# flanggut/smvs

Hardware: NVIDIA H100
Metric: Gauss-Newton Mpix-iters/sec (higher is better)
Workload: dtype f64

## Files before the change

### smvs_b200/csrc/api.cu

```cuda
#include <algorithm>
#include <atomic>
#include <cmath>
#include <cstring>
#include <dlfcn.h>

#include "common.cuh"

namespace smvsb {
std::atomic<uint64_t> g_launches(0);
std::atomic<uint64_t> g_device_launches[SMVSB_MAX_DEVICES];
}

namespace {

thread_local std::string g_last_error = "";

void
quiesce (smvsb_ctx* ctx)
{
    if (ctx == nullptr)
        return;
    if (ctx->copy_stream) cudaStreamSynchronize(ctx->copy_stream);
    if (ctx->stream) cudaStreamSynchronize(ctx->stream);
}
// ... 184 lines not shown
        c->have_color = false;
    }
    for (int k = 0; c->have_color && k < n_sub; ++k)
        if (c->subs[k].w != sub_w[k] || c->subs[k].h != sub_h[k])
            c->have_color = false;
}

void
set_neighbour_tables (smvsb_ctx* c, int n_sub, int const* sub_w,
    int const* sub_h, double const* Mi, double const* ti)
{
    c->n_sub = n_sub;
    std::vector<float const*> ptrs(std::max(n_sub, 1), nullptr);
    std::vector<int> dims(std::max(2 * n_sub, 2), 0);
    std::vector<double> mt(std::max(12 * n_sub, 12), 0.0);
    for (int k = 0; k < n_sub; ++k)
    {
        smvsb::SubViewDev& sv = c->subs[k];
        sv.w = sub_w[k]; sv.h = sub_h[k];
        sv.texels.reserve(static_cast<size_t>(sv.w) * sv.h * SMVSB_NB_STRIDE);
        ptrs[k] = sv.texels.p;
        dims[2 * k] = sv.w; dims[2 * k + 1] = sv.h;
        std::copy(Mi + 9 * k, Mi + 9 * k + 9, mt.begin() + 12 * k);
        std::copy(ti + 3 * k, ti + 3 * k + 3, mt.begin() + 12 * k + 9);
    }
    upload(c, c->sub_ptrs, ptrs.data(), ptrs.size());
    upload(c, c->sub_dims, dims.data(), dims.size());
    upload(c, c->Mt, mt.data(), mt.size());
}

void
upload_color_images (smvsb_ctx* c, float const* main_rgb,
    float const* const* sub_rgb)
{
    upload(c, c->color_main, main_rgb, static_cast<size_t>(c->w) * c->h * 3);
    std::vector<float const*> ptrs(c->n_sub);
    for (int k = 0; k < c->n_sub; ++k)
    {
        upload(c, c->color_subs[k], sub_rgb[k],
            static_cast<size_t>(c->subs[k].w) * c->subs[k].h * 3);
        ptrs[k] = c->color_subs[k].p;
    }
    upload(c, c->color_ptrs, ptrs.data(), ptrs.size());
}

void
ensure_system_buffers (smvsb_ctx* c)
{
    size_t const np = c->n_patches, nn = c->n_nodes;
    c->patch_H.reserve(np * 256);
    c->patch_g.reserve(np * 16);
    c->patch_proc.reserve(np);
    c->H.reserve(nn * 144);
    c->P.reserve(nn * 16);
    c->g.reserve(nn * 4);
    c->x.reserve(nn * 4);
    c->light.reserve(16);
}

void
set_active (smvsb_ctx* c, uint8_t const* active_nodes)
{
    if (active_nodes != nullptr)
        upload(c, c->active, active_nodes, c->n_nodes);
    else
    {
        c->active.reserve(c->n_nodes);
        CUDA_CHECK(cudaMemcpyAsync(c->active.p, c->node_valid.p, c->n_nodes,
            cudaMemcpyDeviceToDevice, c->stream));
    }
}

void
construct (smvsb_ctx* c, double const* light16, double reg, double light_reg)
{
    require(c->have_views && c->have_surface, SMVSB_ERR_STATE,
        "smvsb_set_views and smvsb_set_surface must precede construct");
    if (light16 != nullptr)
    {
        require(c->have_shading, SMVSB_ERR_STATE,
            "lighting given but the main view has no shading image");
        upload(c, c->light, light16, 16);
    }
    ensure_system_buffers(c);
    smvsb::launch_construct(c, light16 != nullptr, reg, light_reg);
    c->have_system = true;
}

void
require_surface_scale (int scale)
{
    require(scale >= 0 && scale <= SMVSB_MAX_SCALE, SMVSB_ERR_INVALID,
        "surface scale out of range (0..8)");
}

void
configure_grid (smvsb_ctx* c, int scale, int npx, int npy, int start_x,
    int start_y)
{
    require_surface_scale(scale);
    require(npx > 0 && npy > 0, SMVSB_ERR_INVALID, "empty patch grid");
    int const ps = 1 << scale;
    int const sampling = sampling_for_scale(scale);
    require(ps % sampling == 0, SMVSB_ERR_INVALID,
        "patch size below sampling");
    int const npos = ps / sampling;
    require(npos == 1 || npos == 2 || npos == 4 || npos == 8
// ... 1203 lines not shown
        {
            require(off.back() <= vis_capacity, SMVSB_ERR_INVALID,
                "vis_ids capacity too small");
            if (off.back() > 0)
                download(c, vis_ids, c->vis_ids.p, off.back());
        }
    });
}

int
smvsb_get_depth (smvsb_ctx* ctx, float* depth_wh)
{
    if (ctx == nullptr) return SMVSB_ERR_INVALID;
    return guarded(ctx, [&]() {
        require(ctx->have_surface && depth_wh, SMVSB_ERR_STATE,
            "no surface set");
        size_t const n = static_cast<size_t>(ctx->w) * ctx->h;
        ctx->image_out.reserve(n * 3);
        smvsb::launch_render_depth(ctx, ctx->image_out.p);
        download(ctx, depth_wh, ctx->image_out.p, n);
    });
}

int
smvsb_get_normals (smvsb_ctx* ctx, float* normals_wh3)
{
    if (ctx == nullptr) return SMVSB_ERR_INVALID;
    return guarded(ctx, [&]() {
        require(ctx->have_surface && normals_wh3, SMVSB_ERR_STATE,
            "no surface set");
        size_t const n = static_cast<size_t>(ctx->w) * ctx->h * 3;
        ctx->image_out.reserve(n);
        smvsb::launch_render_normals(ctx, ctx->image_out.p);
        download(ctx, normals_wh3, ctx->image_out.p, n);
    });
}

int
smvsb_debug_get_system (smvsb_ctx* ctx, double* g, double* Hvals,
    uint64_t* Houter, uint64_t* Hinner, uint64_t* nnzb_h, double* Pvals,
    uint64_t* Pouter, uint64_t* Pinner, uint64_t* nnzb_p)
{
    if (ctx == nullptr) return SMVSB_ERR_INVALID;
    return guarded(ctx, [&]() {
        smvsb_ctx* c = ctx;
        require(c->have_system, SMVSB_ERR_STATE, "no system constructed");
        int const nn = c->n_nodes, ns = c->npx + 1;
        std::vector<uint8_t> active(nn), proc(c->n_patches);
        download(c, active.data(), c->active.p, nn);
        download(c, proc.data(), c->patch_proc.p, c->n_patches);
        if (g)
            download(c, g, c->g.p, static_cast<size_t>(nn) * 4);
        std::vector<double> H, P;
        if (Hvals)
        {
            H.resize(static_cast<size_t>(nn) * 144);
            download(c, H.data(), c->H.p, H.size());
        }
        if (Pvals)
        {
            P.resize(static_cast<size_t>(nn) * 16);
            download(c, P.data(), c->P.p, P.size());
        }
        uint64_t nh = 0, np = 0;
        for (int j = 0; j < nn; ++j)
        {
            if (Houter) Houter[j] = nh;
            if (Pouter) Pouter[j] = np;
            int const jx = j % ns, jy = j / ns;
            if (!c->h_node_valid[j] || !active[j])
                continue;
            for (int dy = -1; dy <= 1; ++dy)
                for (int dx = -1; dx <= 1; ++dx)
                {
                    int const ix = jx + dx, iy = jy + dy;
                    if (ix < 0 || ix > c->npx || iy < 0 || iy > c->npy)
                        continue;
                    int const i = iy * ns + ix;
                    if (!c->h_node_valid[i] || !active[i])
                        continue;
                    bool shared = false;
                    for (int pb = 0; pb < 2 && !shared; ++pb)
                        for (int pa = 0; pa < 2 && !shared; ++pa)
                        {
                            int const px = jx - 1 + pa, py = jy - 1 + pb;
                            if (px < 0 || px >= c->npx || py < 0
                                || py >= c->npy)
                                continue;
                            if (!proc[py * c->npx + px])
                                continue;
                            if (ix >= px && ix <= px + 1 && iy >= py
                                && iy <= py + 1)
                                shared = true;
                        }
                    if (!shared)
                        continue;
                    if (Hvals)
                    {
                        int const k = (-dy + 1) * 3 + (-dx + 1);
                        std::copy(H.begin() + (static_cast<size_t>(i) * 9 + k)
                            * 16, H.begin() + (static_cast<size_t>(i) * 9 + k)
                            * 16 + 16, Hvals + nh * 16);
                    }
                    if (Hinner) Hinner[nh] = static_cast<uint64_t>(i) * 4;
                    nh += 1;
                    if (i == j)
                    {
                        if (Pvals)
                            std::copy(P.begin() + static_cast<size_t>(i) * 16,
                                P.begin() + static_cast<size_t>(i) * 16 + 16,
                                Pvals + np * 16);
                        if (Pinner) Pinner[np] = static_cast<uint64_t>(i) * 4;
                        np += 1;
                    }
                }
// ... 138 lines not shown
```

### smvs_b200/csrc/cg.cu

```cuda
#include <algorithm>

#include "common.cuh"

namespace smvsb {

namespace {

constexpr int CG_THREADS = 256;
constexpr int CG_WARPS = CG_THREADS / 32;
constexpr int CG_QUADS = CG_THREADS / 4;
constexpr int CG_MAX_BLOCKS = 1024;
constexpr int CG_UF = 4;
constexpr int CG_SLOTS = 10;
constexpr int CG_ROW_CACHE = 16;

struct CgView
{
    int n_nodes, npx;
    int grid;
    int pad;
    double err_tol;
    double const* H;
    double const* P;
    double const* g;
    uint16_t const* rowmask;
    uint32_t const* rows;
    unsigned long long const* counts;
    double* x;
    double* r;
    double* d;
    double* d2;
    double* Ad;
    double* z;
    double* partials;
    double* result;
};

struct CgArgs
{
    int n_views;
    int max_iter;
    double q_tol;
    unsigned int* sync;
    CgView v[SMVSB_MAX_BATCH];
};

struct CgState
{
    double r_dot_r, Q0, beta, alpha, tol;
    double* partials;
    int n_rows, passes, done, iters, info;
    int grid;
};

__device__ __forceinline__ void
grid_barrier (unsigned int* counter, unsigned int& epoch)
{
    __syncthreads();
    if (threadIdx.x == 0)
    {
        epoch += 1;
        unsigned int const target = epoch * gridDim.x;
        asm volatile("red.release.gpu.global.add.u32 [%0], 1;"
            :: "l"(counter) : "memory");
        unsigned int v;
        do {
            asm volatile("ld.relaxed.gpu.global.u32 %0, [%1];"
                : "=r"(v) : "l"(counter) : "memory");
        } while (v < target);
        asm volatile("ld.acquire.gpu.global.u32 %0, [%1];"
            : "=r"(v) : "l"(counter) : "memory");
    }
    __syncthreads();
}

__device__ __forceinline__ unsigned long long
policy_evict_first (void)
{
    unsigned long long pol;
    asm("createpolicy.fractional.L2::evict_first.b64 %0, 1.0;" : "=l"(pol));
    return pol;
}

__device__ __forceinline__ void
ld_stream (double const* p, double2& h01, double2& h23)
{
    unsigned long long const pol = policy_evict_first();
    asm volatile("ld.global.L1::no_allocate.L2::cache_hint.v2.f64 "
        "{%0, %1}, [%2], %3;"
        : "=d"(h01.x), "=d"(h01.y) : "l"(p), "l"(pol));
    asm volatile("ld.global.L1::no_allocate.L2::cache_hint.v2.f64 "
        "{%0, %1}, [%2], %3;"
        : "=d"(h23.x), "=d"(h23.y) : "l"(p + 2), "l"(pol));
}

__device__ __forceinline__ double2
ld_vec (double const* p)
{
    return *reinterpret_cast<double2 const*>(p);
}

__device__ __forceinline__ double2
ld_hint (double const* p, unsigned long long policy)
{
    double2 v;
    asm volatile("ld.global.L2::cache_hint.v2.f64 {%0, %1}, [%2], %3;"
        : "=d"(v.x), "=d"(v.y) : "l"(p), "l"(policy));
    return v;
}

__device__ __forceinline__ unsigned long long
policy_evict_last (void)
{
    unsigned long long pol;
    asm volatile("createpolicy.fractional.L2::evict_last.b64 %0, 1.0;"
        : "=l"(pol));
    return pol;
}

template <int NV>
__device__ __forceinline__ void
warp_flush (double (&v)[NV], double* s_red, int view)
{
#pragma unroll
    for (int j = 0; j < NV; ++j)
        for (int off = 16; off > 0; off >>= 1)
            v[j] += __shfl_down_sync(0xffffffffu, v[j], off);
    if ((threadIdx.x & 31) == 0)
    {
#pragma unroll
        for (int j = 0; j < NV; ++j)
            s_red[(view * 3 + j) * CG_WARPS + (threadIdx.x >> 5)] = v[j];
    }
}

template <int NV>
__device__ __forceinline__ void
publish (CgArgs const& a, CgState const* s_state, double const* s_red,
    int first_slot, bool init)
{
    __syncthreads();
    int const t = threadIdx.x;
    if (t < a.n_views * NV)
    {
        int const view = t / NV, j = t % NV;
        CgState const& S = s_state[view];
        if (static_cast<int>(blockIdx.x) < S.grid && (init || !S.done))
        {
            double total = 0.0;
            if (S.passes > 0)
                for (int i = 0; i < CG_WARPS; ++i)
                    total += s_red[(view * 3 + j) * CG_WARPS + i];
            S.partials[(first_slot + j) * CG_MAX_BLOCKS + blockIdx.x] = total;
        }
    }
}

template <int NV>
__device__ __forceinline__ void
all_sums (CgArgs const& a, CgState const* s_state, int first_slot,
    double* s_bcast, bool init)
{
    int const warp = threadIdx.x >> 5, lane = threadIdx.x & 31;
    for (int pair = warp; pair < a.n_views * NV; pair += CG_WARPS)
    {
        int const view = pair / NV, j = pair % NV;
        if (!init && s_state[view].done)
            continue;
        double const* p = s_state[view].partials
            + (first_slot + j) * CG_MAX_BLOCKS;
        int const nb = s_state[view].grid;
        double v = 0.0;
        for (int base = lane; base < nb; base += 32 * 12)
        {
            double t[12];
#pragma unroll
            for (int u = 0; u < 12; ++u)
                t[u] = (base + 32 * u < nb) ? __ldcg(p + base + 32 * u) : 0.0;
#pragma unroll
            for (int u = 0; u < 12; ++u)
                if (base + 32 * u < nb)
                    v += t[u];
        }
        for (int off = 16; off > 0; off >>= 1)
            v += __shfl_down_sync(0xffffffffu, v, off);
        if (lane == 0)
            s_bcast[view * 3 + j] = v;
    }
    __syncthreads();
}

struct PlainVec
{
    double const* v;
    __device__ __forceinline__ void load (int node, double* out) const
    {
        double2 const a = *reinterpret_cast<double2 const*>(
            v + static_cast<size_t>(node) * 4);
        double2 const b = *reinterpret_cast<double2 const*>(
            v + static_cast<size_t>(node) * 4 + 2);
        out[0] = a.x; out[1] = a.y; out[2] = b.x; out[3] = b.y;
    }
};

struct DirVec
{
    double const* z;
    double const* d_old;
    double beta;
    __device__ __forceinline__ void load (int node, double* out) const
    {
        double2 const z0 = ld_vec(z + static_cast<size_t>(node) * 4);
        double2 const z1 = ld_vec(z + static_cast<size_t>(node) * 4 + 2);
        double2 const d0 = ld_vec(d_old + static_cast<size_t>(node) * 4);
        double2 const d1 = ld_vec(d_old + static_cast<size_t>(node) * 4 + 2);
        out[0] = z0.x + d0.x * beta; out[1] = z0.y + d0.y * beta;
        out[2] = z1.x + d1.x * beta; out[3] = z1.y + d1.y * beta;
    }
};

struct StreamRows
{
    double const* H;
    __device__ __forceinline__ double const* row (int node, int rp) const
    {
        return H + static_cast<size_t>(node) * 144 + rp * 4;
    }
    __device__ __forceinline__ void load (double const* p, double2& h01,
        double2& h23) const
    {
        ld_stream(p, h01, h23);
    }
};

constexpr int CG_PIN_STRIDE = 146;
constexpr size_t CG_PIN_BYTES = sizeof(double) * CG_PIN_STRIDE * CG_QUADS;

struct PinnedRows
{
    double const* s;
    __device__ __forceinline__ double const* row (int, int rp) const
    {
        return s + (threadIdx.x >> 2) * CG_PIN_STRIDE + rp * 4;
    }
    __device__ __forceinline__ void load (double const* p, double2& h01,
        double2& h23) const
    {
        h01 = *reinterpret_cast<double2 const*>(p);
        h23 = *reinterpret_cast<double2 const*>(p + 2);
    }
};

template <typename Rows, typename VecOp>
__device__ __forceinline__ double
spmv_row (Rows const& H, int ns, VecOp const& vec, int node, int rp,
    unsigned int mask, double* own)
{
    int const ix = node % ns, iy = node / ns;
    double const* hrow = H.row(node, rp);
    double acc = 0.0;
    own[0] = 0.0; own[1] = 0.0; own[2] = 0.0; own[3] = 0.0;
    if (mask == 0)
        return 0.0;
#pragma unroll
    for (int k = 0; k < 9; ++k)
    {
        if (!((mask >> k) & 1u))
            continue;
        int const jx = ix + (k % 3) - 1, jy = iy + (k / 3) - 1;
        int const nj = jy * ns + jx;
// ... 12 lines not shown
    }
    return acc;
}

__device__ __forceinline__ bool
view_on (CgArgs const& a, CgState const* s_state, int v, bool init)
{
    return static_cast<int>(blockIdx.x) < s_state[v].grid
        && (init || !s_state[v].done) && s_state[v].passes > 0;
}

__device__ __forceinline__ bool
pass_row (CgView const& V, int n_rows, int pass, int& node)
{
    int const q = pass * (V.grid * CG_QUADS) + blockIdx.x * CG_QUADS
        + (threadIdx.x >> 2);
    bool const ok = q < n_rows;
    node = ok ? static_cast<int>(V.rows[q]) : 0;
    return ok;
}

template <int NV>
struct RowCache
{
    static constexpr int PASSES = CG_ROW_CACHE / NV;
    uint32_t node[NV][PASSES][CG_QUADS];
    uint16_t mask[NV][PASSES][CG_QUADS];
};

template <int NV>
__device__ __forceinline__ void
fill_rows (RowCache<NV>& c, CgArgs const& a, CgState const* s_state)
{
    constexpr int N = RowCache<NV>::PASSES * CG_QUADS;
#pragma unroll
    for (int v = 0; v < NV; ++v)
    {
#pragma unroll
        for (int k = 0; k < (N + CG_THREADS - 1) / CG_THREADS; ++k)
        {
            int const e = k * CG_THREADS + threadIdx.x;
            if (e >= N)
                break;
            int const p = e / CG_QUADS, qd = e % CG_QUADS;
            int node = 0;
            unsigned int mask = 0u;
            if (v < a.n_views && static_cast<int>(blockIdx.x) < s_state[v].grid)
            {
                int const q = p * (s_state[v].grid * CG_QUADS)
                    + blockIdx.x * CG_QUADS + qd;
                if (q < s_state[v].n_rows)
                {
                    node = static_cast<int>(a.v[v].rows[q]);
                    mask = a.v[v].rowmask[node];
                }
            }
            c.node[v][p][qd] = static_cast<uint32_t>(node);
            c.mask[v][p][qd] = static_cast<uint16_t>(mask);
        }
    }
}

template <int NV>
__device__ __forceinline__ bool
cached_row (RowCache<NV> const& c, CgView const& V, int v, int n_rows,
    int pass, int& node, unsigned int& mask)
{
    if (pass < RowCache<NV>::PASSES)
    {
        int const qd = threadIdx.x >> 2;
        node = static_cast<int>(c.node[v][pass][qd]);
        mask = c.mask[v][pass][qd];
        return pass * (V.grid * CG_QUADS) + static_cast<int>(blockIdx.x)
            * CG_QUADS + qd < n_rows;
    }
    bool const ok = pass_row(V, n_rows, pass, node);
    mask = ok ? V.rowmask[node] : 0u;
    return ok;
}

template <int NV>
__global__ void __launch_bounds__(CG_THREADS, 2)
cg_kernel (CgArgs const a)
{
    unsigned long long const keep = policy_evict_last();
    __shared__ double s_red[NV * 3 * CG_WARPS];
    __shared__ double s_bcast[NV * 3];
    __shared__ CgState s_state[NV];
    __shared__ double const* s_zptr[NV];
    extern __shared__ __align__(16) double s_pin[];
    __shared__ __align__(8) unsigned long long s_pin_bar;
    __shared__ RowCache<NV> s_rows;
    unsigned int epoch = 0;
    int const quad = threadIdx.x & 28;
    int const rp = threadIdx.x & 3;
    unsigned const pin_bar = static_cast<unsigned>(
        __cvta_generic_to_shared(&s_pin_bar));

    if (threadIdx.x < a.n_views)
    {
        CgView const& V = a.v[threadIdx.x];
        CgState& S = s_state[threadIdx.x];
        S.n_rows = static_cast<int>(V.counts[1]);
        int const per_pass = V.grid * CG_QUADS;
        int const passes = (S.n_rows + per_pass - 1) / per_pass;
        S.passes = ((passes + CG_UF - 1) / CG_UF) * CG_UF;
        S.done = 0; S.iters = 0; S.info = SMVSB_CG_MAX_ITERATIONS;
        S.r_dot_r = 0.0; S.Q0 = 0.0; S.beta = 0.0; S.alpha = 0.0; S.tol = 0.0;
        S.partials = V.partials;
        S.grid = V.grid;
        s_zptr[threadIdx.x] = V.z;
        if (NV == 1)
        {
            int const n_pin = static_cast<int>(blockIdx.x) < V.grid
                ? min(max(S.n_rows - static_cast<int>(blockIdx.x) * CG_QUADS,
                  0), CG_QUADS) : 0;
            if (n_pin > 0)
            {
                asm volatile("mbarrier.init.shared::cta.b64 [%0], %1;"
                    :: "r"(pin_bar), "r"(n_pin));
                asm volatile("fence.mbarrier_init.release.cluster;"
                    ::: "memory");
            }
        }
    }
    __syncthreads();

    bool const pin = NV == 1 && static_cast<int>(blockIdx.x) < s_state[0].grid
        && static_cast<int>(blockIdx.x) * CG_QUADS < s_state[0].n_rows;
    if (NV == 1 && rp == 0)
    {
        int node;
        if (static_cast<int>(blockIdx.x) < s_state[0].grid
            && pass_row(a.v[0], s_state[0].n_rows, 0, node))
        {
            unsigned const dst = static_cast<unsigned>(__cvta_generic_to_shared(
                s_pin + (threadIdx.x >> 2) * CG_PIN_STRIDE));
            double const* src = a.v[0].H + static_cast<size_t>(node) * 144;
            asm volatile("mbarrier.arrive.expect_tx.shared::cta.b64 _, [%0], "
                "%1;" :: "r"(pin_bar), "r"(1152) : "memory");
            asm volatile("cp.async.bulk.shared::cluster.global"
                ".mbarrier::complete_tx::bytes [%0], [%1], %2, [%3];"
                :: "r"(dst), "l"(src), "r"(1152), "r"(pin_bar) : "memory");
        }
    }
    fill_rows(s_rows, a, s_state);

#pragma unroll
    for (int v = 0; v < NV; ++v)
    {
        if (v >= a.n_views || !view_on(a, s_state, v, true))
            continue;
        CgView const& V = a.v[v];
        int const n_rows = s_state[v].n_rows, passes = s_state[v].passes;
        double acc[2] = { 0.0, 0.0 };
        for (int p = 0; p < passes; ++p)
        {
            int node;
            bool const ok = pass_row(V, n_rows, p, node);
            size_t const i = static_cast<size_t>(node) * 4 + rp;
            double const gi = ok ? V.g[i] : 0.0;
            double const ri = -gi;
            double const r0 = __shfl_sync(0xffffffffu, ri, quad);
            double const r1 = __shfl_sync(0xffffffffu, ri, quad + 1);
            double const r2 = __shfl_sync(0xffffffffu, ri, quad + 2);
            double const r3 = __shfl_sync(0xffffffffu, ri, quad + 3);
            if (ok)
            {
                double const* prow = V.P + static_cast<size_t>(node) * 16
                    + rp * 4;
                double2 const p01 = *reinterpret_cast<double2 const*>(prow);
                double2 const p23 = *reinterpret_cast<double2 const*>(prow + 2);
                double const zi = p01.x * r0 + p01.y * r1 + p23.x * r2
                    + p23.y * r3;
                V.r[i] = ri;
                V.z[i] = zi;
                V.d[i] = 0.0;
                V.d2[i] = 0.0;
                V.Ad[i] = 0.0;
                acc[1] += gi * gi;
                acc[0] += zi * ri;
            }
        }
        warp_flush<2>(acc, s_red, v);
    }
    publish<2>(a, s_state, s_red, 0, true);
    grid_barrier(a.sync, epoch);
    all_sums<2>(a, s_state, 0, s_bcast, true);
    if (threadIdx.x < a.n_views)
    {
        CgState& S = s_state[threadIdx.x];
        S.r_dot_r = s_bcast[threadIdx.x * 3 + 0];
        double const gg = s_bcast[threadIdx.x * 3 + 1];
        double const et = a.v[threadIdx.x].err_tol;
        S.tol = (et < 0.0) ? sqrt(gg) * 0.01 : et;
    }
    __syncthreads();

    int iter = 1;
    if (pin)
    {
        unsigned done = 0;
        while (!done)
            asm volatile("{\n.reg .pred p;\n"
                "mbarrier.try_wait.parity.shared::cta.b64 p, [%1], 0;\n"
                "selp.u32 %0, 1, 0, p;\n}"
                : "=r"(done) : "r"(pin_bar) : "memory");
    }
    for (; iter < a.max_iter; ++iter)
    {
        bool const odd = (iter & 1) != 0;
        int const slot = 2 + 4 * (iter & 1);

        {
#pragma unroll
            for (int v = 0; v < NV; ++v)
            {
                if (v >= a.n_views || !view_on(a, s_state, v, false))
                    continue;
                CgView const& V = a.v[v];
                int const n_rows = s_state[v].n_rows;
                int const quads = V.grid * CG_QUADS;
                int const quad0 = blockIdx.x * CG_QUADS + (threadIdx.x >> 2);
                DirVec dir;
                dir.z = s_zptr[v];
                dir.d_old = odd ? V.d : V.d2;
                dir.beta = s_state[v].beta;
                double* d_new = odd ? V.d2 : V.d;
                double acc[1] = { 0.0 };
                int node;
                unsigned int mask;
                cached_row(s_rows, V, v, n_rows, 0, node, mask);
                auto row_pass = [&](auto const& rows, int p)
                {
                    int node_next;
                    unsigned int mask_next;
                    cached_row(s_rows, V, v, n_rows, p + 1, node_next,
                        mask_next);
                    double own[4];
                    size_t const i = static_cast<size_t>(node) * 4 + rp;
                    double const val = spmv_row(rows, V.npx + 1, dir, node, rp,
                        mask, own);
                    node = node_next;
                    mask = mask_next;
                    double const di = (rp == 0) ? own[0] : (rp == 1) ? own[1]
                        : (rp == 2) ? own[2] : own[3];
                    V.Ad[i] = val;
                    d_new[i] = di;
                    acc[0] += val * di;
                };
                int q = quad0, p = 0;
                if (NV == 1 && q < n_rows)
                {
                    row_pass(PinnedRows{ s_pin }, p);
                    q += quads;
                    ++p;
                }
                for (; q < n_rows; q += quads, ++p)
                    row_pass(StreamRows{ V.H }, p);
                warp_flush<1>(acc, s_red, v);
            }
            publish<1>(a, s_state, s_red, slot, false);
        }
        grid_barrier(a.sync, epoch);
        all_sums<1>(a, s_state, slot, s_bcast, false);
        if (threadIdx.x < a.n_views && !s_state[threadIdx.x].done)
            s_state[threadIdx.x].alpha = s_state[threadIdx.x].r_dot_r
                / s_bcast[threadIdx.x * 3];
        __syncthreads();

#pragma unroll
        for (int v = 0; v < NV; ++v)
        {
            if (v >= a.n_views || !view_on(a, s_state, v, false))
                continue;
            CgView const& V = a.v[v];
            int const n_rows = s_state[v].n_rows;
            int const passes = s_state[v].passes;
            double const alpha = s_state[v].alpha;
            double const* d_new = odd ? V.d2 : V.d;
            double acc[3] = { 0.0, 0.0, 0.0 };
            int nodes[CG_UF];
            bool oks[CG_UF];
            unsigned int unused;
#pragma unroll
            for (int u = 0; u < CG_UF; ++u)
                oks[u] = cached_row(s_rows, V, v, n_rows, u, nodes[u], unused);
            for (int p = 0; p < passes; p += CG_UF)
            {
                int nodes_next[CG_UF];
                bool oks_next[CG_UF];
#pragma unroll
                for (int u = 0; u < CG_UF; ++u)
                    oks_next[u] = cached_row(s_rows, V, v, n_rows,
                        p + CG_UF + u, nodes_next[u], unused);

                double xv[CG_UF], rv[CG_UF], gv[CG_UF];
                double2 p01[CG_UF], p23[CG_UF];
#pragma unroll
                for (int u = 0; u < CG_UF; ++u)
                {
                    xv[u] = 0.0; rv[u] = 0.0; gv[u] = 0.0;
                    p01[u] = make_double2(0, 0); p23[u] = p01[u];
                    if (oks[u])
                    {
                        size_t const i = static_cast<size_t>(nodes[u]) * 4 + rp;
                        double const dn = d_new[i], ad = V.Ad[i];
                        gv[u] = V.g[i];
                        xv[u] = V.x[i]; rv[u] = V.r[i];
                        double const* prow = V.P
                            + static_cast<size_t>(nodes[u]) * 16 + rp * 4;
                        p01[u] = ld_hint(prow, keep);
                        p23[u] = ld_hint(prow + 2, keep);
                        xv[u] += dn * alpha; rv[u] -= ad * alpha;
                    }
                }
#pragma unroll
                for (int u = 0; u < CG_UF; ++u)
                {
                    double const q0 = __shfl_sync(0xffffffffu, rv[u], quad);
                    double const q1 = __shfl_sync(0xffffffffu, rv[u], quad + 1);
                    double const q2 = __shfl_sync(0xffffffffu, rv[u], quad + 2);
                    double const q3 = __shfl_sync(0xffffffffu, rv[u], quad + 3);
                    if (oks[u])
                    {
                        size_t const i = static_cast<size_t>(nodes[u]) * 4 + rp;
                        double const zi = p01[u].x * q0 + p01[u].y * q1
                            + p23[u].x * q2 + p23[u].y * q3;
                        V.x[i] = xv[u]; V.r[i] = rv[u];
                        V.z[i] = zi;
                        acc[0] += rv[u] * rv[u];
                        acc[1] += xv[u] * (rv[u] - gv[u]);
                        acc[2] += zi * rv[u];
                    }
                }
#pragma unroll
                for (int u = 0; u < CG_UF; ++u)
                {
                    nodes[u] = nodes_next[u];
                    oks[u] = oks_next[u];
                }
            }
            warp_flush<3>(acc, s_red, v);
        }
        publish<3>(a, s_state, s_red, slot + 1, false);
        grid_barrier(a.sync, epoch);
        all_sums<3>(a, s_state, slot + 1, s_bcast, false);

        if (threadIdx.x < a.n_views && !s_state[threadIdx.x].done)
        {
            CgState& S = s_state[threadIdx.x];
            double const new_rr = s_bcast[threadIdx.x * 3 + 0];
            double const xbr = s_bcast[threadIdx.x * 3 + 1];
            double const new_zr = s_bcast[threadIdx.x * 3 + 2];
            bool stop = false;
            if (new_rr < S.tol)
                stop = true;
            else
            {
                double const Q1 = -1.0 * xbr;
                double const zeta = iter * (Q1 - S.Q0) / Q1;
                if (zeta < a.q_tol)
                    stop = true;
                else
                {
                    S.Q0 = Q1;
                    S.beta = new_zr / S.r_dot_r;
                    S.r_dot_r = new_zr;
                }
            }
            if (stop)
            {
                S.done = 1;
                S.iters = iter;
                S.info = SMVSB_CG_CONVERGENCE;
            }
        }
        __syncthreads();
        bool all_done = true;
        for (int v = 0; v < a.n_views; ++v)
            all_done = all_done && (s_state[v].done != 0);
        if (all_done)
            break;
    }

    if (blockIdx.x == 0 && threadIdx.x < a.n_views)
    {
        CgState const& S = s_state[threadIdx.x];
        double* res = a.v[threadIdx.x].result;
        res[0] = S.done ? S.iters : iter;
        res[1] = S.info;
        res[2] = isnan(__ldcg(a.v[threadIdx.x].x)) ? 1.0 : 0.0;
    }
}

__global__ void __launch_bounds__(256)
cg_mark_kernel (int npx, int npy, uint8_t const* __restrict__ node_valid,
    uint8_t const* __restrict__ active, uint16_t* __restrict__ rowmask,
    uint32_t* __restrict__ block_rows, unsigned long long* __restrict__ counts)
{
    int const node = blockIdx.x * blockDim.x + threadIdx.x;
    int const ns = npx + 1;
    unsigned int m = 0;
    if (node < ns * (npy + 1) && node_valid[node] && active[node])
    {
        int const ix = node % ns, iy = node / ns;
        for (int k = 0; k < 9; ++k)
        {
            int const jx = ix + (k % 3) - 1, jy = iy + (k / 3) - 1;
            if (jx < 0 || jx > npx || jy < 0 || jy > npy)
                continue;
            int const nj = jy * ns + jx;
            if (node_valid[nj] && active[nj])
                m |= 1u << k;
        }
    }
    if (node < ns * (npy + 1))
        rowmask[node] = static_cast<uint16_t>(m);
    unsigned int const blocks = __reduce_add_sync(0xffffffffu, __popc(m));
    int const rows = __syncthreads_count(m != 0);
    if ((threadIdx.x & 31) == 0)
        atomicAdd(counts, static_cast<unsigned long long>(blocks));
    if (threadIdx.x == 0)
    {
        block_rows[blockIdx.x] = rows;
        atomicAdd(counts + 1, static_cast<unsigned long long>(rows));
    }
}

__global__ void __launch_bounds__(256)
cg_list_kernel (int n_nodes, uint16_t const* __restrict__ rowmask,
    uint32_t const* __restrict__ block_off, uint32_t* __restrict__ rows)
{
    __shared__ uint32_t s_warp[8];
    int const node = blockIdx.x * blockDim.x + threadIdx.x;
    bool const on = node < n_nodes && rowmask[node] != 0;
    unsigned int const ballot = __ballot_sync(0xffffffffu, on);
    int const lane = threadIdx.x & 31, warp = threadIdx.x >> 5;
    if (lane == 0)
        s_warp[warp] = __popc(ballot);
    __syncthreads();
    uint32_t before = block_off[blockIdx.x];
    for (int w = 0; w < warp; ++w)
        before += s_warp[w];
    before += __popc(ballot & ((1u << lane) - 1u));
    if (on)
        rows[before] = node;
}

__global__ void
spmv_kernel (int n_nodes, int npx, double const* __restrict__ H,
    uint16_t const* __restrict__ rowmask, double const* __restrict__ x,
    double* __restrict__ y)
{
    int const i = blockIdx.x * blockDim.x + threadIdx.x;
    if (i >= n_nodes * 4)
        return;
    PlainVec vec;
    vec.v = x;
    StreamRows const rows{ H };
    double own[4];
    y[i] = spmv_row(rows, npx + 1, vec, i >> 2, i & 3, rowmask[i >> 2], own);
}

void
mark_system (smvsb_ctx* c)
{
    int const nb = (c->n_nodes + 255) / 256;
    c->cg_rowmask.reserve(c->n_nodes);
    c->cg_row_list.reserve(c->n_nodes);
    c->cg_block_rows.reserve(2 * static_cast<size_t>(nb) + 1);
    c->cg_counts.reserve(2);
    CUDA_CHECK(cudaMemsetAsync(c->cg_counts.p, 0,
        2 * sizeof(unsigned long long), c->stream));
    cg_mark_kernel<<<nb, 256, 0, c->stream>>>(c->npx, c->npy,
        c->node_valid.p, c->active.p, c->cg_rowmask.p, c->cg_block_rows.p,
        c->cg_counts.p);
    CUDA_CHECK(cudaGetLastError());
    launch_exclusive_scan(c, c->cg_block_rows.p, c->cg_block_rows.p + nb, nb);
    cg_list_kernel<<<nb, 256, 0, c->stream>>>(c->n_nodes, c->cg_rowmask.p,
        c->cg_block_rows.p + nb, c->cg_row_list.p);
    smvsb::count_launches(c, 2);
    CUDA_CHECK(cudaGetLastError());
}

}

void
launch_spmv (smvsb_ctx* c, double const* x, double* y)
{
    mark_system(c);
    int const n = c->n_nodes * 4;
    spmv_kernel<<<(n + 255) / 256, 256, 0, c->stream>>>(c->n_nodes, c->npx,
        c->H.p, c->cg_rowmask.p, x, y);
    smvsb::count_launches(c, 1);
    CUDA_CHECK(cudaGetLastError());
}

void
cg_enqueue (smvsb_ctx* const* cs, int n, int max_iter, double err_tol,
    double q_tol)
{
    if (n < 1 || n > SMVSB_MAX_BATCH)
        throw Error(SMVSB_ERR_INVALID, "batch size out of range");
    smvsb_ctx* lead = cs[0];
    void const* kernel = nullptr;
    if (n == 1)
        kernel = (void const*)cg_kernel<1>;
    else if (n == 2)
        kernel = (void const*)cg_kernel<2>;
    else if (n <= 4)
        kernel = (void const*)cg_kernel<4>;
    else
        kernel = (void const*)cg_kernel<8>;

    size_t const dyn_smem = (n == 1) ? CG_PIN_BYTES : 0;
    if (n == 1)
    {
        cudaFuncAttributes fa;
        CUDA_CHECK(cudaFuncGetAttributes(&fa, kernel));
        int smem_sm = 0, reserved = 0;
        CUDA_CHECK(cudaDeviceGetAttribute(&smem_sm,
            cudaDevAttrMaxSharedMemoryPerMultiprocessor, lead->device));
        CUDA_CHECK(cudaDeviceGetAttribute(&reserved,
            cudaDevAttrReservedSharedMemoryPerBlock, lead->device));
        size_t const need = 2 * (dyn_smem + fa.sharedSizeBytes + reserved);
        int const carveout = static_cast<int>(std::min<size_t>(100,
            (100 * need + smem_sm - 1) / smem_sm));
        CUDA_CHECK(cudaFuncSetAttribute(kernel,
            cudaFuncAttributeMaxDynamicSharedMemorySize,
            static_cast<int>(dyn_smem)));
        CUDA_CHECK(cudaFuncSetAttribute(kernel,
            cudaFuncAttributePreferredSharedMemoryCarveout, carveout));
    }
    int per_sm = 0;
    CUDA_CHECK(cudaOccupancyMaxActiveBlocksPerMultiprocessor(&per_sm,
        kernel, CG_THREADS, dyn_smem));
    if (per_sm < 1)
        throw Error(SMVSB_ERR_CUDA, "cg_kernel does not fit on an SM");
    if (n == 1 && per_sm < 2)
        throw Error(SMVSB_ERR_CUDA, "cg_kernel<1> fits only "
            + std::to_string(per_sm) + " CTA per SM, needs 2");
    int const grid_max = std::min(lead->num_sms * std::min(per_sm, 2),
        CG_MAX_BLOCKS);

    CgArgs a;
    a.n_views = n; a.max_iter = max_iter; a.q_tol = q_tol;
    lead->cg_sync.reserve(1);
    a.sync = lead->cg_sync.p;
    int grid = 1;
    for (int k = 0; k < n; ++k)
    {
        smvsb_ctx* c = cs[k];
        size_t const nn = static_cast<size_t>(c->n_nodes) * 4;
        c->x.reserve(nn); c->r.reserve(nn); c->d.reserve(nn);
        c->d2.reserve(nn); c->Ad.reserve(nn); c->z.reserve(nn);
        c->cg_partials.reserve(static_cast<size_t>(CG_SLOTS) * CG_MAX_BLOCKS);
        c->cg_result.reserve(16);
        mark_system(c);
        CUDA_CHECK(cudaMemsetAsync(c->x.p, 0, nn * sizeof(double),
            c->stream));
        CgView& V = a.v[k];
        V.n_nodes = c->n_nodes; V.npx = c->npx; V.pad = 0;
        int const need = static_cast<int>((nn + CG_THREADS - 1) / CG_THREADS);
        V.grid = std::max(1, std::min(grid_max, need));
        grid = std::max(grid, V.grid);
        V.err_tol = err_tol;
        V.H = c->H.p; V.P = c->P.p; V.g = c->g.p;
        V.rowmask = c->cg_rowmask.p; V.rows = c->cg_row_list.p;
        V.counts = c->cg_counts.p;
        V.x = c->x.p; V.r = c->r.p; V.d = c->d.p; V.d2 = c->d2.p;
        V.Ad = c->Ad.p; V.z = c->z.p;
        V.partials = c->cg_partials.p; V.result = c->cg_result.p;
    }
    CUDA_CHECK(cudaMemsetAsync(a.sync, 0, sizeof(unsigned int), lead->stream));
    void* params[] = { &a };
    CUDA_CHECK(cudaLaunchCooperativeKernel(kernel, dim3(grid),
        dim3(CG_THREADS), params, dyn_smem, lead->stream));
    smvsb::count_launches(lead, 1);
    CUDA_CHECK(cudaGetLastError());
    for (int k = 0; k < n; ++k)
    {
        smvsb_ctx* c = cs[k];
        CUDA_CHECK(cudaMemcpyAsync(c->pinned->cg, c->cg_result.p,
            3 * sizeof(double), cudaMemcpyDeviceToHost, c->stream));
        CUDA_CHECK(cudaMemcpyAsync(c->pinned->cg_counts, c->cg_counts.p,
            2 * sizeof(unsigned long long), cudaMemcpyDeviceToHost,
            c->stream));
    }
}

void
cg_collect (smvsb_ctx* c, int* iters, int* info, bool* x0_nan)
{
    double const* res = c->pinned->cg;
    c->cg_blocks = c->pinned->cg_counts[0];
    c->cg_rows = c->pinned->cg_counts[1];
    if (iters) *iters = static_cast<int>(res[0]);
    if (info) *info = static_cast<int>(res[1]);
    if (x0_nan) *x0_nan = (res[2] != 0.0);
}

void
run_cg (smvsb_ctx* c, int max_iter, double err_tol, double q_tol, int* iters,
    int* info, bool* x0_nan)
{
    smvsb_ctx* cs[1] = { c };
    cg_enqueue(cs, 1, max_iter, err_tol, q_tol);
    CUDA_CHECK(cudaStreamSynchronize(c->stream));
    cg_collect(c, iters, info, x0_nan);
}

}
```

### smvs_b200/csrc/common.cuh

```cuda
#ifndef SMVSB_COMMON_CUH
#define SMVSB_COMMON_CUH

#include <cuda_runtime.h>

#include <atomic>
#include <cstdint>
#include <cstdio>
#include <string>
#include <vector>

#include "../../include/smvs_b200.h"

#define SMVSB_MAX_SUBS 32
#define SMVSB_MAX_SCALE 8
#define SMVSB_NB_STRIDE 8
#define SMVSB_NUM_EVENTS 6

#define CUDA_CHECK(call)                                                     \
    do {                                                                     \
        cudaError_t e__ = (call);                                            \
        if (e__ != cudaSuccess)                                              \
            throw smvsb::Error(SMVSB_ERR_CUDA, std::string(#call) + ": "     \
                + cudaGetErrorString(e__));                                  \
    } while (0)

namespace smvsb {

struct Error
{
    int code;
    std::string msg;
    Error (int c, std::string const& m) : code(c), msg(m) {}
};

template <typename T>
struct DevBuf
{
    T* p = nullptr;
    size_t cap = 0;

    DevBuf (void) = default;
    DevBuf (DevBuf const&) = delete;
    DevBuf& operator= (DevBuf const&) = delete;
    ~DevBuf (void) { if (p) cudaFree(p); }

    void reserve (size_t n)
    {
        if (n <= cap)
            return;
        if (p) { cudaFree(p); p = nullptr; cap = 0; }
        cudaError_t e = cudaMalloc(&p, n * sizeof(T));
        if (e != cudaSuccess)
        {
            p = nullptr;
            throw Error(SMVSB_ERR_ALLOC, std::string("cudaMalloc of ")
                + std::to_string(n * sizeof(T)) + " bytes: "
                + cudaGetErrorString(e));
        }
        cap = n;
    }

    void release (void)
    {
        if (p) cudaFree(p);
        p = nullptr;
        cap = 0;
    }

    size_t bytes (void) const { return cap * sizeof(T); }
// ... 39 lines not shown
};

}

struct smvsb_ctx
{
    int device = 0;
    cudaStream_t stream = nullptr;
    cudaEvent_t ev[SMVSB_NUM_EVENTS] = {};
    cudaStream_t copy_stream = nullptr;
    cudaEvent_t ev_copied[2] = {}, ev_consumed[2] = {};
    std::string last_error;
    uint64_t launches = 0;
    int num_sms = 0;

    bool have_views = false;
    int w = 0, h = 0, n_sub = 0;
    double flen = 0, inv_flen = 0;
    smvsb::DevBuf<float> main_grad, main_shading, main_shading_grad;
    bool have_shading = false;
    smvsb::SubViewDev subs[SMVSB_MAX_SUBS];
    smvsb::DevBuf<float const*> sub_ptrs;
    smvsb::DevBuf<int> sub_dims;
    smvsb::DevBuf<double> Mt;
    smvsb::DevBuf<uint8_t> stage_u8;
    smvsb::DevBuf<uint8_t> stage_u8b;
    smvsb::DevBuf<float> stage_a, stage_b;
    smvsb::DevBuf<float> view_in, view_texels, view_out;

    bool have_surface = false;
    int scale = 0, ps = 0, sampling = 0, npos = 0;
    int npx = 0, npy = 0, start_x = 0, start_y = 0;
    int n_nodes = 0, n_patches = 0;
    smvsb::DevBuf<double> nodes;
    smvsb::DevBuf<uint8_t> node_valid, patch_valid, vis_ids;
    smvsb::DevBuf<uint32_t> vis_off;
    smvsb::DevBuf<uint8_t> active, active_new;
    smvsb::DevBuf<double> basis_s, basis_f;
    std::vector<uint8_t> h_node_valid, h_patch_valid;

    smvsb::DevBuf<float> init_depth;
    smvsb::DevBuf<double> nodes_tmp;
    smvsb::DevBuf<uint8_t> node_valid_tmp;
    smvsb::DevBuf<uint8_t> u8_main;
    smvsb::DevBuf<uint8_t> u8_subs[SMVSB_MAX_SUBS];
    smvsb::DevBuf<float> guide;

    bool have_system = false;
    smvsb::DevBuf<double> patch_H;
    smvsb::DevBuf<double> patch_g;
    smvsb::DevBuf<uint8_t> patch_proc;
    smvsb::DevBuf<double> H;
    smvsb::DevBuf<double> P;
    smvsb::DevBuf<double> g;
    smvsb::DevBuf<double> light;

    smvsb::DevBuf<double> x, r, d, d2, z, Ad;
    size_t x_count = 0;
    smvsb::DevBuf<double> cg_partials;
    smvsb::DevBuf<uint16_t> cg_rowmask;
    smvsb::DevBuf<uint32_t> cg_row_list, cg_block_rows;
    smvsb::DevBuf<unsigned long long> cg_counts;
    uint64_t cg_blocks = 0, cg_rows = 0;
    smvsb::PinnedResults* pinned = nullptr;
    smvsb::DevBuf<unsigned int> cg_sync;
    smvsb::DevBuf<double> cg_result;

    smvsb::DevBuf<double> patch_shift;
    smvsb::DevBuf<double> upd_partials, upd_result;
    smvsb::DevBuf<unsigned long long> counters;

    smvsb::DevBuf<unsigned int> zbuf, vis_mask;
    smvsb::DevBuf<unsigned long long> zoff;
    smvsb::DevBuf<float> sgm_depth;
    bool have_color = false;
    smvsb::DevBuf<float> color_main;
    smvsb::DevBuf<float> color_subs[SMVSB_MAX_SUBS];
    smvsb::DevBuf<float const*> color_ptrs;
    smvsb::DevBuf<short4> rim_lists;
    int rim_ps = 0;
    int rim_off[9] = {};
    smvsb::DevBuf<uint32_t> vis_counts;

    smvsb::DevBuf<double> light_partials;

    smvsb::DevBuf<float> image_out;
};

namespace smvsb {

#define SMVSB_MAX_DEVICES 64
extern std::atomic<uint64_t> g_launches;
extern std::atomic<uint64_t> g_device_launches[SMVSB_MAX_DEVICES];

inline void
count_device_launches (int device, int n)
{
    g_launches += n;
    if (device >= 0 && device < SMVSB_MAX_DEVICES)
        g_device_launches[device] += n;
}

inline void
count_launches (smvsb_ctx* c, int n)
{
    c->launches += n;
    count_device_launches(c->device, n);
}

inline void
// ... 132 lines not shown
```

### smvs_b200/csrc/gn_construct.cu

```cuda
#include "gn_math.cuh"
#include "patch_eval.cuh"

namespace smvsb {

namespace {

constexpr int K1_THREADS = 128;
constexpr int AS_STRIDE = 27;

__host__ __device__ inline void
hermite (double t, double* b0, double* b1, double* b2)
{
    double const t2 = t * t, t3 = t2 * t;
    b0[0] = 2 * t3 - 3 * t2 + 1;
    b0[1] = -2 * t3 + 3 * t2;
    b0[2] = t3 - 2 * t2 + t;
    b0[3] = t3 - t2;
    b1[0] = 6 * t2 - 6 * t;
    b1[1] = -6 * t2 + 6 * t;
    b1[2] = 3 * t2 - 4 * t + 1;
    b1[3] = 3 * t2 - 2 * t;
    b2[0] = 12 * t - 6;
    b2[1] = -12 * t + 6;
    b2[2] = 6 * t - 4;
// ... 470 lines not shown
    int const ns = sf.npx + 1;
    int const ix = node % ns, iy = node / ns;
    int const dx = k % 3 - 1, dy = k / 3 - 1;
    int const jx = ix + dx, jy = iy + dy;

    double acc[4] = {0.0, 0.0, 0.0, 0.0};
    double gacc = 0.0;
    bool const row_on = sf.node_valid[node] && sf.active[node];
    bool col_on = false;
    if (jx >= 0 && jx <= sf.npx && jy >= 0 && jy <= sf.npy)
    {
        int const nj = jy * ns + jx;
        col_on = sf.node_valid[nj] && sf.active[nj];
    }

    if (row_on)
    {
#pragma unroll
        for (int pb = 0; pb < 2; ++pb)
#pragma unroll
            for (int pa = 0; pa < 2; ++pa)
            {
                int const ppx = ix - 1 + pa, ppy = iy - 1 + pb;
                if (ppx < 0 || ppx >= sf.npx || ppy < 0 || ppy >= sf.npy)
                    continue;
                int const patch = ppy * sf.npx + ppx;
                if (!patch_proc[patch])
                    continue;
                int const li = (1 - pa) + 2 * (1 - pb);
                if (k == 4)
                    gacc += patch_g[static_cast<size_t>(patch) * 16
                        + li * 4 + rp];
                int const ljx = dx + 1 - pa, ljy = dy + 1 - pb;
                if (!col_on || ljx < 0 || ljx > 1 || ljy < 0 || ljy > 1)
                    continue;
                int const lj = ljx + 2 * ljy;
                double const* src = patch_H + (static_cast<size_t>(patch) * 16
                    + li * 4 + rp) * 16 + lj * 4;
                double2 const a = *reinterpret_cast<double2 const*>(src);
                double2 const b = *reinterpret_cast<double2 const*>(src + 2);
                acc[0] += a.x; acc[1] += a.y; acc[2] += b.x; acc[3] += b.y;
            }
    }
    double2* dst = reinterpret_cast<double2*>(
        H + (static_cast<size_t>(node) * 9 + k) * 16 + rp * 4);
    dst[0] = make_double2(acc[0], acc[1]);
    dst[1] = make_double2(acc[2], acc[3]);
    if (k == 4)
        g[static_cast<size_t>(node) * 4 + rp] = gacc;
}

__global__ void
gn_precond_kernel (SurfaceDev const sf, double const* __restrict__ H,
    double* __restrict__ P)
{
    int const node = blockIdx.x * blockDim.x + threadIdx.x;
    if (node >= sf.n_nodes)
        return;
    double A[16], out[16];
    bool const on = sf.node_valid[node] && sf.active[node];
    double const* src = H + (static_cast<size_t>(node) * 9 + 4) * 16;
#pragma unroll
    for (int i = 0; i < 16; ++i) A[i] = on ? src[i] : 0.0;
    if (on)
    {
        bool ok = ldl_inverse4(A, out);
        if (ok)
        {
            bool nan = false;
#pragma unroll
            for (int i = 0; i < 16; ++i) nan = nan || isnan(out[i]);
            ok = !nan;
        }
        if (!ok)
        {
#pragma unroll
            for (int i = 0; i < 16; ++i) out[i] = A[i];
        }
    }
    else
    {
#pragma unroll
        for (int i = 0; i < 16; ++i) out[i] = 0.0;
    }
    double* dst = P + static_cast<size_t>(node) * 16;
#pragma unroll
    for (int i = 0; i < 16; ++i) dst[i] = out[i];
}

void
launch_construct (smvsb_ctx* c, bool use_light, double reg, double light_reg)
{
    ConstructArgs a;
    a.s = surface_args(c);
    a.regularization = reg;
    a.light_surf_regularization = light_reg;
    a.light = use_light ? c->light.p : nullptr;
    a.patch_H = c->patch_H.p;
    a.patch_g = c->patch_g.p;
    a.patch_proc = c->patch_proc.p;

    int const S = c->npos * c->npos;
    auto blocks = [&](int ppb) { return (c->n_patches + ppb - 1) / ppb; };
    switch (S)
    {
    case 1:
        gn_patch_kernel<1><<<blocks(8), K1_THREADS, 0, c->stream>>>(a); break;
    case 4:
        gn_patch_kernel<4><<<blocks(8), K1_THREADS, 0, c->stream>>>(a); break;
    case 16:
    {
        gn_patch_kernel<16><<<blocks(8), K1_THREADS, 0, c->stream>>>(a);
        break;
    }
    case 64:
        gn_patch_kernel<64><<<blocks(2), K1_THREADS, 0, c->stream>>>(a); break;
    case 256:
        gn_patch_kernel<256><<<blocks(1), K1_THREADS, 0, c->stream>>>(a); break;
    case 1024:
        gn_patch_kernel<1024><<<blocks(1), K1_THREADS, 0, c->stream>>>(a);
        break;
    case 4096:
        gn_patch_kernel<4096><<<blocks(1), K1_THREADS, 0, c->stream>>>(a);
        break;
    default:
        throw Error(SMVSB_ERR_INVALID, "unsupported samples per patch");
    }
    CUDA_CHECK(cudaGetLastError());

    int const n_thr = c->n_nodes * 36;
    gn_assemble_kernel<<<(n_thr + 287) / 288, 288, 0, c->stream>>>(a.s,
        c->patch_H.p, c->patch_g.p, c->patch_proc.p, c->H.p, c->g.p);
    CUDA_CHECK(cudaGetLastError());
    gn_precond_kernel<<<(c->n_nodes + 127) / 128, 128, 0, c->stream>>>(a.s,
        c->H.p, c->P.p);
    CUDA_CHECK(cudaGetLastError());
    smvsb::count_launches(c, 3);
}

}
```

Measured before the change: 158.1.

## Pack symmetric preconditioner to upper triangle and recompute CG direction in update pass

Stores the 4x4 block-Jacobi preconditioner as 10 packed upper-triangle doubles instead of 16. A per-node fallback flag is encoded in the high bit of the CG row list, so nodes whose inverse failed read the H diagonal block directly. It also drops the d2 double buffer: the SpMV no longer writes the new direction, and the update pass recomputes d = z + beta*d with an FMA and writes it back. Both changes cut memory traffic in a bandwidth-bound CG, at the cost of scalar gathered loads for P and extra index masking.

Result: faster. 160.1, median of 6 (+1.3%).

```diff
diff --git a/smvs_b200/csrc/api.cu b/smvs_b200/csrc/api.cu
--- a/smvs_b200/csrc/api.cu
+++ b/smvs_b200/csrc/api.cu
@@ -260,7 +260,8 @@
     c->patch_g.reserve(np * 16);
     c->patch_proc.reserve(np);
     c->H.reserve(nn * 144);
-    c->P.reserve(nn * 16);
+    c->P.reserve(nn * SMVSB_P_PACKED);
+    c->P_fallback.reserve(nn);
     c->g.reserve(nn * 4);
     c->x.reserve(nn * 4);
     c->light.reserve(16);
@@ -1570,15 +1571,33 @@
         if (g)
             download(c, g, c->g.p, static_cast<size_t>(nn) * 4);
         std::vector<double> H, P;
-        if (Hvals)
+        if (Hvals || Pvals)
         {
             H.resize(static_cast<size_t>(nn) * 144);
             download(c, H.data(), c->H.p, H.size());
         }
         if (Pvals)
         {
+            std::vector<double> packed(static_cast<size_t>(nn)
+                * SMVSB_P_PACKED);
+            std::vector<uint8_t> fallback(nn);
+            download(c, packed.data(), c->P.p, packed.size());
+            download(c, fallback.data(), c->P_fallback.p, fallback.size());
             P.resize(static_cast<size_t>(nn) * 16);
-            download(c, P.data(), c->P.p, P.size());
+            for (size_t i = 0; i < static_cast<size_t>(nn); ++i)
+            {
+                double* dst = P.data() + i * 16;
+                if (fallback[i])
+                {
+                    std::copy(H.begin() + (i * 9 + 4) * 16,
+                        H.begin() + (i * 9 + 4) * 16 + 16, dst);
+                    continue;
+                }
+                double const* src = packed.data() + i * SMVSB_P_PACKED;
+                for (int r = 0, o = 0; r < 4; ++r)
+                    for (int col = r; col < 4; ++col, ++o)
+                        dst[r * 4 + col] = dst[col * 4 + r] = src[o];
+            }
         }
         uint64_t nh = 0, np = 0;
         for (int j = 0; j < nn; ++j)
diff --git a/smvs_b200/csrc/cg.cu b/smvs_b200/csrc/cg.cu
--- a/smvs_b200/csrc/cg.cu
+++ b/smvs_b200/csrc/cg.cu
@@ -1,4 +1,5 @@
 #include <algorithm>
+#include <climits>
 
 #include "common.cuh"
 
@@ -29,7 +30,6 @@
     double* x;
     double* r;
     double* d;
-    double* d2;
     double* Ad;
     double* z;
     double* partials;
@@ -100,15 +100,6 @@
     return *reinterpret_cast<double2 const*>(p);
 }
 
-__device__ __forceinline__ double2
-ld_hint (double const* p, unsigned long long policy)
-{
-    double2 v;
-    asm volatile("ld.global.L2::cache_hint.v2.f64 {%0, %1}, [%2], %3;"
-        : "=d"(v.x), "=d"(v.y) : "l"(p), "l"(policy));
-    return v;
-}
-
 __device__ __forceinline__ unsigned long long
 policy_evict_last (void)
 {
@@ -116,6 +107,32 @@
     asm volatile("createpolicy.fractional.L2::evict_last.b64 %0, 1.0;"
         : "=l"(pol));
     return pol;
+}
+
+constexpr uint32_t CG_FALLBACK = 0x80000000u;
+
+__device__ __forceinline__ int
+entry_node (int entry)
+{
+    return entry & INT_MAX;
+}
+
+__device__ __forceinline__ void
+ld_prow (CgView const& V, int entry, int rp, unsigned long long policy,
+    double (&p)[4])
+{
+    int const node = entry_node(entry);
+    bool const fallback = entry < 0;
+    double const* base = fallback
+        ? V.H + static_cast<size_t>(node) * 144 + 4 * 16 + rp * 4
+        : V.P + static_cast<size_t>(node) * SMVSB_P_PACKED;
+    unsigned int const offs = fallback ? 0x3210u : rp == 0 ? 0x3210u
+        : rp == 1 ? 0x6541u : rp == 2 ? 0x8752u : 0x9863u;
+#pragma unroll
+    for (int c = 0; c < 4; ++c)
+        asm volatile("ld.global.L2::cache_hint.f64 %0, [%1], %2;"
+            : "=d"(p[c]) : "l"(base + ((offs >> (4 * c)) & 15u)),
+              "l"(policy));
 }
 
 template <int NV>
@@ -214,8 +231,10 @@
         double2 const z1 = ld_vec(z + static_cast<size_t>(node) * 4 + 2);
         double2 const d0 = ld_vec(d_old + static_cast<size_t>(node) * 4);
         double2 const d1 = ld_vec(d_old + static_cast<size_t>(node) * 4 + 2);
-        out[0] = z0.x + d0.x * beta; out[1] = z0.y + d0.y * beta;
-        out[2] = z1.x + d1.x * beta; out[3] = z1.y + d1.y * beta;
+        out[0] = __fma_rn(d0.x, beta, z0.x);
+        out[1] = __fma_rn(d0.y, beta, z0.y);
+        out[2] = __fma_rn(d1.x, beta, z1.x);
+        out[3] = __fma_rn(d1.y, beta, z1.y);
     }
 };
 
@@ -334,7 +353,7 @@
                 if (q < s_state[v].n_rows)
                 {
                     node = static_cast<int>(a.v[v].rows[q]);
-                    mask = a.v[v].rowmask[node];
+                    mask = a.v[v].rowmask[entry_node(node)];
                 }
             }
             c.node[v][p][qd] = static_cast<uint32_t>(node);
@@ -357,7 +376,7 @@
             * CG_QUADS + qd < n_rows;
     }
     bool const ok = pass_row(V, n_rows, pass, node);
-    mask = ok ? V.rowmask[node] : 0u;
+    mask = ok ? V.rowmask[entry_node(node)] : 0u;
     return ok;
 }
 
@@ -418,7 +437,8 @@
         {
             unsigned const dst = static_cast<unsigned>(__cvta_generic_to_shared(
                 s_pin + (threadIdx.x >> 2) * CG_PIN_STRIDE));
-            double const* src = a.v[0].H + static_cast<size_t>(node) * 144;
+            double const* src = a.v[0].H
+                + static_cast<size_t>(entry_node(node)) * 144;
             asm volatile("mbarrier.arrive.expect_tx.shared::cta.b64 _, [%0], "
                 "%1;" :: "r"(pin_bar), "r"(1152) : "memory");
             asm volatile("cp.async.bulk.shared::cluster.global"
@@ -438,9 +458,9 @@
         double acc[2] = { 0.0, 0.0 };
         for (int p = 0; p < passes; ++p)
         {
-            int node;
-            bool const ok = pass_row(V, n_rows, p, node);
-            size_t const i = static_cast<size_t>(node) * 4 + rp;
+            int entry;
+            bool const ok = pass_row(V, n_rows, p, entry);
+            size_t const i = static_cast<size_t>(entry_node(entry)) * 4 + rp;
             double const gi = ok ? V.g[i] : 0.0;
             double const ri = -gi;
             double const r0 = __shfl_sync(0xffffffffu, ri, quad);
@@ -449,16 +469,13 @@
             double const r3 = __shfl_sync(0xffffffffu, ri, quad + 3);
             if (ok)
             {
-                double const* prow = V.P + static_cast<size_t>(node) * 16
-                    + rp * 4;
-                double2 const p01 = *reinterpret_cast<double2 const*>(prow);
-                double2 const p23 = *reinterpret_cast<double2 const*>(prow + 2);
-                double const zi = p01.x * r0 + p01.y * r1 + p23.x * r2
-                    + p23.y * r3;
+                double pr[4];
+                ld_prow(V, entry, rp, keep, pr);
+                double const zi = pr[0] * r0 + pr[1] * r1 + pr[2] * r2
+                    + pr[3] * r3;
                 V.r[i] = ri;
                 V.z[i] = zi;
                 V.d[i] = 0.0;
-                V.d2[i] = 0.0;
                 V.Ad[i] = 0.0;
                 acc[1] += gi * gi;
                 acc[0] += zi * ri;
@@ -491,7 +508,6 @@
     }
     for (; iter < a.max_iter; ++iter)
     {
-        bool const odd = (iter & 1) != 0;
         int const slot = 2 + 4 * (iter & 1);
 
         {
@@ -506,29 +522,28 @@
                 int const quad0 = blockIdx.x * CG_QUADS + (threadIdx.x >> 2);
                 DirVec dir;
                 dir.z = s_zptr[v];
-                dir.d_old = odd ? V.d : V.d2;
+                dir.d_old = V.d;
                 dir.beta = s_state[v].beta;
-                double* d_new = odd ? V.d2 : V.d;
                 double acc[1] = { 0.0 };
-                int node;
+                int entry;
                 unsigned int mask;
-                cached_row(s_rows, V, v, n_rows, 0, node, mask);
+                cached_row(s_rows, V, v, n_rows, 0, entry, mask);
                 auto row_pass = [&](auto const& rows, int p)
                 {
-                    int node_next;
+                    int entry_next;
                     unsigned int mask_next;
-                    cached_row(s_rows, V, v, n_rows, p + 1, node_next,
+                    cached_row(s_rows, V, v, n_rows, p + 1, entry_next,
                         mask_next);
                     double own[4];
+                    int const node = entry_node(entry);
                     size_t const i = static_cast<size_t>(node) * 4 + rp;
                     double const val = spmv_row(rows, V.npx + 1, dir, node, rp,
                         mask, own);
-                    node = node_next;
+                    entry = entry_next;
                     mask = mask_next;
                     double const di = (rp == 0) ? own[0] : (rp == 1) ? own[1]
                         : (rp == 2) ? own[2] : own[3];
                     V.Ad[i] = val;
-                    d_new[i] = di;
                     acc[0] += val * di;
                 };
                 int q = quad0, p = 0;
@@ -560,40 +575,43 @@
             int const n_rows = s_state[v].n_rows;
             int const passes = s_state[v].passes;
             double const alpha = s_state[v].alpha;
-            double const* d_new = odd ? V.d2 : V.d;
+            double const beta = s_state[v].beta;
             double acc[3] = { 0.0, 0.0, 0.0 };
-            int nodes[CG_UF];
+            int entries[CG_UF];
             bool oks[CG_UF];
             unsigned int unused;
 #pragma unroll
             for (int u = 0; u < CG_UF; ++u)
-                oks[u] = cached_row(s_rows, V, v, n_rows, u, nodes[u], unused);
+                oks[u] = cached_row(s_rows, V, v, n_rows, u, entries[u],
+                    unused);
             for (int p = 0; p < passes; p += CG_UF)
             {
-                int nodes_next[CG_UF];
+                int entries_next[CG_UF];
                 bool oks_next[CG_UF];
 #pragma unroll
                 for (int u = 0; u < CG_UF; ++u)
                     oks_next[u] = cached_row(s_rows, V, v, n_rows,
-                        p + CG_UF + u, nodes_next[u], unused);
+                        p + CG_UF + u, entries_next[u], unused);
 
                 double xv[CG_UF], rv[CG_UF], gv[CG_UF];
-                double2 p01[CG_UF], p23[CG_UF];
+                double pr[CG_UF][4];
 #pragma unroll
                 for (int u = 0; u < CG_UF; ++u)
                 {
                     xv[u] = 0.0; rv[u] = 0.0; gv[u] = 0.0;
-                    p01[u] = make_double2(0, 0); p23[u] = p01[u];
+                    pr[u][0] = 0.0; pr[u][1] = 0.0;
+                    pr[u][2] = 0.0; pr[u][3] = 0.0;
                     if (oks[u])
                     {
-                        size_t const i = static_cast<size_t>(nodes[u]) * 4 + rp;
-                        double const dn = d_new[i], ad = V.Ad[i];
+                        size_t const i
+                            = static_cast<size_t>(entry_node(entries[u])) * 4
+                            + rp;
+                        double const dn = __fma_rn(V.d[i], beta, V.z[i]);
+                        double const ad = V.Ad[i];
                         gv[u] = V.g[i];
                         xv[u] = V.x[i]; rv[u] = V.r[i];
-                        double const* prow = V.P
-                            + static_cast<size_t>(nodes[u]) * 16 + rp * 4;
-                        p01[u] = ld_hint(prow, keep);
-                        p23[u] = ld_hint(prow + 2, keep);
+                        ld_prow(V, entries[u], rp, keep, pr[u]);
+                        V.d[i] = dn;
                         xv[u] += dn * alpha; rv[u] -= ad * alpha;
                     }
                 }
@@ -606,9 +624,11 @@
                     double const q3 = __shfl_sync(0xffffffffu, rv[u], quad + 3);
                     if (oks[u])
                     {
-                        size_t const i = static_cast<size_t>(nodes[u]) * 4 + rp;
-                        double const zi = p01[u].x * q0 + p01[u].y * q1
-                            + p23[u].x * q2 + p23[u].y * q3;
+                        size_t const i
+                            = static_cast<size_t>(entry_node(entries[u])) * 4
+                            + rp;
+                        double const zi = pr[u][0] * q0 + pr[u][1] * q1
+                            + pr[u][2] * q2 + pr[u][3] * q3;
                         V.x[i] = xv[u]; V.r[i] = rv[u];
                         V.z[i] = zi;
                         acc[0] += rv[u] * rv[u];
@@ -619,7 +639,7 @@
 #pragma unroll
                 for (int u = 0; u < CG_UF; ++u)
                 {
-                    nodes[u] = nodes_next[u];
+                    entries[u] = entries_next[u];
                     oks[u] = oks_next[u];
                 }
             }
@@ -712,6 +732,7 @@
 
 __global__ void __launch_bounds__(256)
 cg_list_kernel (int n_nodes, uint16_t const* __restrict__ rowmask,
+    uint8_t const* __restrict__ p_fallback,
     uint32_t const* __restrict__ block_off, uint32_t* __restrict__ rows)
 {
     __shared__ uint32_t s_warp[8];
@@ -727,7 +748,7 @@
         before += s_warp[w];
     before += __popc(ballot & ((1u << lane) - 1u));
     if (on)
-        rows[before] = node;
+        rows[before] = p_fallback[node] ? node | CG_FALLBACK : node;
 }
 
 __global__ void
@@ -761,7 +782,7 @@
     CUDA_CHECK(cudaGetLastError());
     launch_exclusive_scan(c, c->cg_block_rows.p, c->cg_block_rows.p + nb, nb);
     cg_list_kernel<<<nb, 256, 0, c->stream>>>(c->n_nodes, c->cg_rowmask.p,
-        c->cg_block_rows.p + nb, c->cg_row_list.p);
+        c->P_fallback.p, c->cg_block_rows.p + nb, c->cg_row_list.p);
     smvsb::count_launches(c, 2);
     CUDA_CHECK(cudaGetLastError());
 }
@@ -836,7 +857,7 @@
         smvsb_ctx* c = cs[k];
         size_t const nn = static_cast<size_t>(c->n_nodes) * 4;
         c->x.reserve(nn); c->r.reserve(nn); c->d.reserve(nn);
-        c->d2.reserve(nn); c->Ad.reserve(nn); c->z.reserve(nn);
+        c->Ad.reserve(nn); c->z.reserve(nn);
         c->cg_partials.reserve(static_cast<size_t>(CG_SLOTS) * CG_MAX_BLOCKS);
         c->cg_result.reserve(16);
         mark_system(c);
@@ -851,7 +872,7 @@
         V.H = c->H.p; V.P = c->P.p; V.g = c->g.p;
         V.rowmask = c->cg_rowmask.p; V.rows = c->cg_row_list.p;
         V.counts = c->cg_counts.p;
-        V.x = c->x.p; V.r = c->r.p; V.d = c->d.p; V.d2 = c->d2.p;
+        V.x = c->x.p; V.r = c->r.p; V.d = c->d.p;
         V.Ad = c->Ad.p; V.z = c->z.p;
         V.partials = c->cg_partials.p; V.result = c->cg_result.p;
     }
diff --git a/smvs_b200/csrc/common.cuh b/smvs_b200/csrc/common.cuh
--- a/smvs_b200/csrc/common.cuh
+++ b/smvs_b200/csrc/common.cuh
@@ -15,6 +15,7 @@
 #define SMVSB_MAX_SCALE 8
 #define SMVSB_NB_STRIDE 8
 #define SMVSB_NUM_EVENTS 6
+#define SMVSB_P_PACKED 10
 
 #define CUDA_CHECK(call)                                                     \
     do {                                                                     \
@@ -160,10 +161,11 @@
     smvsb::DevBuf<uint8_t> patch_proc;
     smvsb::DevBuf<double> H;
     smvsb::DevBuf<double> P;
+    smvsb::DevBuf<uint8_t> P_fallback;
     smvsb::DevBuf<double> g;
     smvsb::DevBuf<double> light;
 
-    smvsb::DevBuf<double> x, r, d, d2, z, Ad;
+    smvsb::DevBuf<double> x, r, d, z, Ad;
     size_t x_count = 0;
     smvsb::DevBuf<double> cg_partials;
     smvsb::DevBuf<uint16_t> cg_rowmask;
diff --git a/smvs_b200/csrc/gn_construct.cu b/smvs_b200/csrc/gn_construct.cu
--- a/smvs_b200/csrc/gn_construct.cu
+++ b/smvs_b200/csrc/gn_construct.cu
@@ -546,13 +546,14 @@
 
 __global__ void
 gn_precond_kernel (SurfaceDev const sf, double const* __restrict__ H,
-    double* __restrict__ P)
+    double* __restrict__ P, uint8_t* __restrict__ P_fallback)
 {
     int const node = blockIdx.x * blockDim.x + threadIdx.x;
     if (node >= sf.n_nodes)
         return;
     double A[16], out[16];
     bool const on = sf.node_valid[node] && sf.active[node];
+    bool fallback = false;
     double const* src = H + (static_cast<size_t>(node) * 9 + 4) * 16;
 #pragma unroll
     for (int i = 0; i < 16; ++i) A[i] = on ? src[i] : 0.0;
@@ -566,20 +567,21 @@
             for (int i = 0; i < 16; ++i) nan = nan || isnan(out[i]);
             ok = !nan;
         }
-        if (!ok)
-        {
-#pragma unroll
-            for (int i = 0; i < 16; ++i) out[i] = A[i];
-        }
-    }
-    else
+        fallback = !ok;
+    }
+    if (!on || fallback)
     {
 #pragma unroll
         for (int i = 0; i < 16; ++i) out[i] = 0.0;
     }
-    double* dst = P + static_cast<size_t>(node) * 16;
-#pragma unroll
-    for (int i = 0; i < 16; ++i) dst[i] = out[i];
+    double2* dst = reinterpret_cast<double2*>(
+        P + static_cast<size_t>(node) * SMVSB_P_PACKED);
+    dst[0] = make_double2(out[0], out[1]);
+    dst[1] = make_double2(out[2], out[3]);
+    dst[2] = make_double2(out[5], out[6]);
+    dst[3] = make_double2(out[7], out[10]);
+    dst[4] = make_double2(out[11], out[15]);
+    P_fallback[node] = fallback ? 1 : 0;
 }
 
 void
@@ -627,7 +629,7 @@
         c->patch_H.p, c->patch_g.p, c->patch_proc.p, c->H.p, c->g.p);
     CUDA_CHECK(cudaGetLastError());
     gn_precond_kernel<<<(c->n_nodes + 127) / 128, 128, 0, c->stream>>>(a.s,
-        c->H.p, c->P.p);
+        c->H.p, c->P.p, c->P_fallback.p);
     CUDA_CHECK(cudaGetLastError());
     smvsb::count_launches(c, 3);
 }
```
